# JianCao92/speaker-diarization

Hardware: AMD Instinct MI355X
Metric: diarized audio throughput (CD gw/BIC + CL hi/BIC) (higher is better)
Workload: dtype f64

## Files before the change

speaker-diarization_amd/csrc/spkd_cluster.hpp:

```cpp
#pragma once
#include "spkd_device.hpp"
#include "spkd_quad.hpp"
#include "spkd_tri.hpp"
#include "../../include/spkd.h"

namespace spkd {

constexpr double MAXINT_F = 9223372036854775808.0;
constexpr double PEN_UNIT = 39.0 + 0.5 * 39.0 * 40.0;
constexpr int AUX = 3 * DA;
constexpr int ERR_DEGENERATE_MERGE = 2;

__device__ __forceinline__ unsigned long long dkey(double v) {
    unsigned long long b = (unsigned long long)__double_as_longlong(v);
    return (b >> 63) ? ~b : (b | 0x8000000000000000ull);
}
__device__ __forceinline__ double dkey_inv(unsigned long long k) {
    unsigned long long b = (k >> 63) ? (k & 0x7fffffffffffffffull) : ~k;
    return __longlong_as_double((long long)b);
}
template <bool MAXOP>
__device__ __forceinline__ unsigned wave_red_u32(unsigned x) {
    auto op = [](unsigned a, unsigned b) { return MAXOP ? (a > b ? a : b) : (a < b ? a : b); };
    x = op(x, (unsigned)__builtin_amdgcn_update_dpp((int)x, (int)x, 0xB1, 0xf, 0xf, false));
// ... 485 lines not shown
                wmin = (wmin != wmin || d < wmin) ? d : wmin;
            }
        }
        if (variant == 1 && lane_id() == 0) {
            if (wmax == wmax) atomicMax(stat_max + p, dkey(wmax));
            if (wmin == wmin) atomicMin(stat_min + p, dkey(wmin));
        }
        return;
    }
    double* row = Dm + ra * N;
    for (int64_t base = ra + 1 + 4 * wave; base < N; base += 4 * MX_WAVES) {
        int64_t rc = base + L.m;
        const bool valid = rc < N;
        rc = valid ? rc : N - 1;
        const double det = quad_pair_det<TWO>(kind, ldsA, nA, A, ex + (off + rc) * QREC, pk + (off + rc) * REC, false, L, err);
        if (valid && L.t == 0) row[rc] = det;
    }
    __syncthreads();
    double wmax = __builtin_nan(""), wmin = __builtin_nan("");
    for (int64_t c = ra + 1 + threadIdx.x; c < N; c += MX_WAVES * WAVE) {
        const double det = row[c];
        const double nC = pk[(off + c) * REC + REC - 1];
        const double d = finish_distance(kind, lambdac, nA, ldA, nC, ld[off + c], log(det));
        row[c] = d;
        if (variant == 1) {
            Dm[c * N + ra] = d;
            if (stat_valid(d)) {
                wmax = (wmax != wmax || d > wmax) ? d : wmax;
                wmin = (wmin != wmin || d < wmin) ? d : wmin;
            }
        }
    }
    if (variant == 1) {
        const unsigned long long kmax = wave_red_u64<true>(wmax == wmax ? dkey(wmax) : 0ull);
        const unsigned long long kmin = wave_red_u64<false>(wmin == wmin ? dkey(wmin) : ~0ull);
        if (lane_id() == 0) {
            if (kmax != 0ull) atomicMax(stat_max + p, kmax);
            if (kmin != ~0ull) atomicMin(stat_min + p, kmin);
        }
    }
}

constexpr int AHC_WAVES = 8;
constexpr int AHC_TPB = AHC_WAVES * WAVE;

#ifdef SPKD_PROFILE
__device__ unsigned long long g_step_prof[8];
__device__ unsigned long long g_ahc_prof[8];
constexpr int AHC_SPAN_PROBS = 4096;
__device__ unsigned long long g_ahc_span[2 * AHC_SPAN_PROBS];
#endif
constexpr int NO_COL = 0x7fffffff;
constexpr int AHC_MAX_N = 65536;


struct RowMin { double mv; int mc, nc; };

template <class Alive>
__device__ __forceinline__ RowMin scan_row(const double* __restrict__ row, long long N, Alive alive,
                                           long long sub_col, double sub_val, int lane) {
    double mv = __builtin_huge_val();
    int mc = NO_COL, nc = NO_COL;
    for (long long c0 = 0; c0 < N; c0 += 4 * WAVE) {
        double v[4];
        int a[4];
#pragma unroll
        for (int u = 0; u < 4; ++u) {
            const long long c = c0 + u * WAVE + lane;
            const long long cc = c < N ? c : N - 1;
            a[u] = (c < N) ? (alive(cc) ? 1 : 0) : 0;
            v[u] = row[cc];
        }
#pragma unroll
        for (int u = 0; u < 4; ++u) {
            const long long cl = c0 + u * WAVE + lane;
            const int c = (int)cl;
            if (!a[u]) continue;
            const double x = (cl == sub_col) ? sub_val : v[u];
            if (x != x) { if (c < nc) nc = c; continue; }
            if (x < mv || (x == mv && c < mc)) { mv = x; mc = c; }
        }
    }
    unsigned long long okey;
    unsigned oc;
    wave_argmin_key(mc != NO_COL ? dkey(mv) : ~0ull, (unsigned)mc, okey, oc);
    RowMin r;
    r.mv = okey != ~0ull ? dkey_inv(okey) : __builtin_huge_val();
    r.mc = okey != ~0ull ? (int)oc : NO_COL;
    r.nc = __any(nc != NO_COL) ? (int)wave_red_u32<false>((unsigned)nc) : NO_COL;
    return r;
}

__device__ __forceinline__ bool row_cache_after_merge(int variant, double d, int sa, int sb,
                                                      double& rm, int& ra, int& rn) {
    if (variant != 1) return ra == sb || rn == sb;
    const bool nan_hit = rn == sa || rn == sb;
    if (ra == sa || ra == sb || nan_hit) {
        if (nan_hit || !(d < rm)) return true;
        rm = d; ra = sa;
    } else if (d != d) {
        if (sa < rn) rn = sa;
    } else if (d < rm || (d == rm && sa < ra)) {
        rm = d; ra = sa;
    }
    return false;
}
// ... 24 lines not shown
    double mx = s_tmax[0];
    if (tid == 0) {
        for (int w = 1; w < AHC_WAVES; ++w) {
            const double x = s_tmax[w];
            if (mx == mx) mx = (x != x) ? x : (x > mx ? x : mx);
        }
    }
    return mx;
}

__device__ __forceinline__ void refresh_rows(const double* __restrict__ Dm, long long N,
                                             const int32_t* __restrict__ al, int32_t* __restrict__ dirty,
                                             double* __restrict__ rmin, int32_t* __restrict__ rarg,
                                             int32_t* __restrict__ rnan, unsigned long long* masks,
                                             int tid, int wave, int lane) {
    const long long n_chunks = (N + WAVE - 1) / WAVE;
    for (long long ch = wave; ch < n_chunks; ch += AHC_WAVES) {
        const long long rl = ch * WAVE + lane;
        const long long rc = rl < N ? rl : N - 1;
        const int fa = al[rc], fd = dirty[rc];
        const unsigned long long mk = __ballot(rl < N && fa && fd);
        if (lane == 0) masks[ch] = mk;
    }
    __syncthreads();
    int ord = 0;
    for (long long ch = 0; ch < n_chunks; ++ch) {
        const long long r0 = ch * WAVE;
        unsigned long long todo = masks[ch];
        while (todo) {
            const int b = __builtin_ctzll(todo);
            todo &= todo - 1;
            if ((ord++ & (AHC_WAVES - 1)) != wave) continue;
            const long long r = r0 + b;
            const RowMin e = scan_row(Dm + r * N, N, [&](long long c) { return al[c] != 0; }, -1, 0.0, lane);
            if (lane == 0) { rmin[r] = e.mv; rarg[r] = e.mc; rnan[r] = e.nc; dirty[r] = 0; }
#ifdef SPKD_PROFILE
            if (lane == 0) atomicAdd(&g_ahc_prof[0], 1ull);
#endif
        }
    }
}

template <bool TWO>
__global__ __launch_bounds__(AHC_TPB) void k_ahc(
        double* __restrict__ ex, double* __restrict__ pk, const int64_t* __restrict__ seg_off,
        int variant, int kind, int max_spk, double lambdac, double threshold,
        double* __restrict__ ld, double* __restrict__ aux,
        double* __restrict__ mat, const int64_t* __restrict__ mat_off,
        int32_t* __restrict__ alive, double* __restrict__ tmp,
        double* __restrict__ rmin_all, int32_t* __restrict__ rcache_all,
        int32_t* __restrict__ out_n, int32_t* __restrict__ out_a, int32_t* __restrict__ out_b,
        double* __restrict__ out_d, unsigned long long* stat_max, unsigned long long* stat_min,
        double* __restrict__ final_max, double* __restrict__ final_min, int* err,
        double* pinv_ws, const int32_t* __restrict__ prob_of_block) {
    extern __shared__ int32_t ids[];
    __shared__ double ldsA[QREC];
    __shared__ unsigned long long red3[AHC_WAVES][3];
    __shared__ unsigned long long s_masks[AHC_MAX_N / WAVE];
    __shared__ int s_cnt[2];
    __shared__ int s_nids;
    __shared__ int s_next;
    __shared__ double s_tmax[AHC_WAVES];
    const int tid = threadIdx.x, lane = lane_id(), wave = tid >> 6;
    const QuadLane L = quad_lane();
    const int p = prob_of_block ? prob_of_block[blockIdx.x] : (int)blockIdx.x;
#ifdef SPKD_PROFILE
    if (tid == 0 && p < AHC_SPAN_PROBS) g_ahc_span[2 * p] = wall_clock64();
#endif
    const int64_t off = seg_off[p];
    const long long N = seg_off[p + 1] - off;
    double* Dm = mat + mat_off[p];
    int32_t* al = alive + off;
    double* ldp = ld + off;
    double* tp = tmp + off;
    double* rmin = rmin_all + off;
    int32_t* rarg = rcache_all + 3 * off;
    int32_t* rnan = rarg + N;
    int32_t* dirty = rnan + N;
    for (long long c = tid; c < N; c += AHC_TPB) { al[c] = 1; dirty[c] = 1; }
    __syncthreads();
    long long m = N;
    int n_merges = 0;
    const long long INF_IDX = 0x7fffffffffffffffLL;
    double fmin = 0.0;
#ifdef SPKD_PROFILE
    unsigned long long ahc_acc[5] = {0ull, 0ull, 0ull, 0ull, 0ull}, ahc_t = clock64();
#define AHC_TICK(i) do { const unsigned long long now_ = clock64(); ahc_acc[i] += now_ - ahc_t; ahc_t = now_; } while (0)
#else
#define AHC_TICK(i) ((void)0)
#endif
    while (true) {
        refresh_rows(Dm, N, al, dirty, rmin, rarg, rnan, s_masks, tid, wave, lane);
        __syncthreads();
        AHC_TICK(0);
        unsigned long long kb = ~0ull, ib = ~0ull, inan = ~0ull;
        for (long long r = tid; r < N; r += AHC_TPB) {
            if (!al[r]) continue;
            const double v = rmin[r];
            const int c = rarg[r], nc = rnan[r];
            if (nc != NO_COL) { const unsigned long long l = (unsigned long long)(r * N + nc); inan = l < inan ? l : inan; }
            if (c != NO_COL) {
                const unsigned long long kv = dkey(v);
                if (kv < kb) { kb = kv; ib = (unsigned long long)(r * N + c); }
            }
        }
        {
            const unsigned long long wk = wave_red_u64<false>(kb);
            const unsigned long long wi = wave_red_u64<false>(kb == wk ? ib : ~0ull);
            const unsigned long long wn = __any(inan != ~0ull) ? wave_red_u64<false>(inan) : ~0ull;
            if (lane == 0) { red3[wave][0] = wk; red3[wave][1] = wi; red3[wave][2] = wn; }
        }
        __syncthreads();
        unsigned long long bk = red3[0][0], bi = red3[0][1], bn = red3[0][2];
#pragma unroll
        for (int w = 1; w < AHC_WAVES; ++w) {
            const unsigned long long ok = red3[w][0], oi = red3[w][1], on = red3[w][2];
            const bool t = ok < bk || (ok == bk && oi < bi);
            bk = t ? ok : bk; bi = t ? oi : bi;
            bn = on < bn ? on : bn;
        }
        const bool has_nan = bn != ~0ull;
        const double mind = has_nan ? __builtin_nan("") : (bi != ~0ull ? dkey_inv(bk) : __builtin_huge_val());
        const long long index = has_nan ? (long long)bn : (bi != ~0ull ? (long long)bi : INF_IDX);
        fmin = mind;
        const bool go = (mind <= threshold) || (max_spk > 0 && m > max_spk);
        if (!go) break;
        AHC_TICK(1);
        const long long r0 = index / N, c0 = index - r0 * N;
        if (r0 == c0) {
            if (tid == 0) atomicOr(err, ERR_DEGENERATE_MERGE);
            break;
        }
        const long long sa = r0 < c0 ? r0 : c0, sb = r0 < c0 ? c0 : r0;
        if (tid < 2) s_cnt[tid] = 0;
        if (tid == 0) { s_nids = 1; s_next = 0; }
        __syncthreads();
        {
            int ca = 0, cb = 0;
            for (long long c = tid; c < sb; c += AHC_TPB) {
                if (al[c]) { cb++; if (c < sa) ca++; }
            }
            ca = __builtin_amdgcn_readlane(wave_scan_i32(ca), WAVE - 1);
            cb = __builtin_amdgcn_readlane(wave_scan_i32(cb), WAVE - 1);
            if (lane == 0 && ca) atomicAdd(&s_cnt[0], ca);
            if (lane == 0 && cb) atomicAdd(&s_cnt[1], cb);
        }
        __syncthreads();
        if (tid == 0) {
            const int64_t o = off + n_merges;
            out_a[o] = s_cnt[0]; out_b[o] = s_cnt[1]; out_d[o] = mind;
            al[sb] = 0;
            ids[0] = (int32_t)sa;
        }
        n_merges++;
        m--;
#ifdef SPKD_PROFILE
        if (tid == 0) atomicAdd(&g_ahc_prof[1], 1ull);
#endif
        double* A = ex + (off + sa) * QREC;
        const double* B = ex + (off + sb) * QREC;
        {
            double* Ap = pk + (off + sa) * REC;
            const double* Bp = pk + (off + sb) * REC;
            constexpr int NQ = (QREC + AHC_TPB - 1) / AHC_TPB, NP = (REC + AHC_TPB - 1) / AHC_TPB;
            double qa[NQ], qb[NQ], pa[NP], pb[NP];
#pragma unroll
            for (int u = 0; u < NQ; ++u) {
                const int e = tid + u * AHC_TPB;
                qa[u] = A[e < QREC ? e : 0]; qb[u] = B[e < QREC ? e : 0];
            }
#pragma unroll
            for (int u = 0; u < NP; ++u) {
                const int e = tid + u * AHC_TPB;
                pa[u] = Ap[e < REC ? e : 0]; pb[u] = Bp[e < REC ? e : 0];
            }
#pragma unroll
            for (int u = 0; u < NQ; ++u) {
                const int e = tid + u * AHC_TPB;
                const double v = qa[u] + qb[u];
                if (e < QREC) { A[e] = v; ldsA[e] = v; }
            }
#pragma unroll
            for (int u = 0; u < NP; ++u) {
                const int e = tid + u * AHC_TPB;
                if (e < REC) Ap[e] = pa[u] + pb[u];
            }
        }
        __syncthreads();
        for (long long c0 = 0; c0 < N; c0 += AHC_TPB) {
            const long long c = c0 + tid;
            const bool take = c < N && c != sa && al[c < N ? c : N - 1];
            const unsigned long long mk = __ballot(take);
            int base = 0;
            if (lane == 0 && mk) base = atomicAdd(&s_nids, __popcll(mk));
            base = __shfl(base, 0);
            if (take) ids[base + __popcll(mk & ((1ull << lane) - 1ull))] = (int32_t)c;
        }
        __syncthreads();
        AHC_TICK(2);
        const int nids = s_nids;
        const double nA = ldsA[QREC_COUNT_AT];
        if (kind == SPKD_KL2) {
            if (wave == 0) kl2_aux_from_qr(ldsA, aux + (off + sa) * AUX, pinv_ws);
        } else {
            for (;;) {
                int q4 = 0;
                if (lane == 0) q4 = atomicAdd(&s_next, 1);
                const int base = 4 * __builtin_amdgcn_readfirstlane(q4);
                if (base >= nids) break;
                int k = base + L.m;
                const bool valid = k < nids;
                k = valid ? k : nids - 1;
                const int32_t slot = ids[k];
                const double v = quad_pair_det<TWO>(kind, ldsA, nA, A, ex + (off + slot) * QREC, pk + (off + slot) * REC, k == 0, L, err);
                if (valid && L.t == 0) {
                    if (k == 0) ldp[sa] = log(v); else tp[slot] = v;
                }
            }
        }
        __syncthreads();
        AHC_TICK(3);
        double wmax = __builtin_nan(""), wmin = __builtin_nan("");
        const double ldA = ldp[sa];
        for (long long c = tid; c < N; c += AHC_TPB) {
            if (c == sa || !al[c]) continue;
            double d;
            if (kind == SPKD_KL2) {
                d = kl2_from_aux_serial(aux + (off + sa) * AUX, aux + (off + c) * AUX);
            } else {
                const double nC = qr_count(ex + (off + c) * QREC);
                d = finish_distance(kind, lambdac, nA, ldA, nC, ldp[c], log(tp[c]));
            }
            Dm[sa * N + c] = d;
            const double rm0 = rmin[c];
            const int ra0 = rarg[c], rn0 = rnan[c];
            double rm = rm0;
            int ra = ra0, rn = rn0;
            if (variant == 1) Dm[c * N + sa] = d;
            if (row_cache_after_merge(variant, d, (int)sa, (int)sb, rm, ra, rn)) dirty[c] = 1;
            else {
                if (rm != rm0 || ra != ra0) { rmin[c] = rm; rarg[c] = ra; }
                if (rn != rn0) rnan[c] = rn;
            }
            if (variant == 1 && stat_valid(d)) {
                wmax = (wmax != wmax || d > wmax) ? d : wmax;
                wmin = (wmin != wmin || d < wmin) ? d : wmin;
            }
        }
        if (tid == 0) dirty[sa] = 1;
        if (variant == 1) {
            const unsigned long long kmax = wave_red_u64<true>(wmax == wmax ? dkey(wmax) : 0ull);
            const unsigned long long kmin = wave_red_u64<false>(wmin == wmin ? dkey(wmin) : ~0ull);
            if (lane == 0) {
                if (kmax != 0ull) atomicMax(stat_max + p, kmax);
                if (kmin != ~0ull) atomicMin(stat_min + p, kmin);
            }
        }
        __syncthreads();
        AHC_TICK(4);
    }
#ifdef SPKD_PROFILE
    if (tid == 0) for (int i = 0; i < 5; ++i) atomicAdd(&g_ahc_prof[2 + i], ahc_acc[i]);
#endif
    const double mx = final_matrix_max(Dm, N, [&](long long c) { return al[c] != 0; }, s_tmax, tid);
    if (tid == 0) {
        out_n[p] = n_merges;
        final_max[p] = mx;
        final_min[p] = fmin;
#ifdef SPKD_PROFILE
        if (p < AHC_SPAN_PROBS) g_ahc_span[2 * p + 1] = wall_clock64();
#endif
    }
}

constexpr int STEP_WAVES = 4;
constexpr int STEP_WIDE_FROM = 1024;
constexpr int STEP_PARTNERS = 4 * STEP_WAVES - 1;
constexpr int ALIVE_ROUND = 0x7fffffff;
constexpr int STEP_MAX_N = 16384;
constexpr int STEP_IDX_SHIFT = 14;

struct StepState {
    int32_t done, n_merges;
    long long psa;
    double fmin;
    double diag;
};

__host__ __device__ inline unsigned long long step_slot_word(int round, int new_slot, int old_slot) {
    return ((unsigned long long)(unsigned)round << 40) | ((unsigned long long)(unsigned)new_slot << 20) |
           (unsigned long long)(unsigned)old_slot;
}
__device__ __forceinline__ int step_slot_of(unsigned long long w, int k) {
    return ((int)(w >> 40) < k) ? (int)((w >> 20) & 0xfffffull) : (int)(w & 0xfffffull);
}

struct StepSel {
    double rmin, newrow;
    int32_t rarg, rnan, death, pad;
};

struct StepArrays {
    double* ex;
    double* pk;
    double* exm;
    double* pkm;
    int32_t* death;
    StepSel* sel2;
    unsigned long long* sw;
    double* cnt;
    StepState* state2;
// ... 574 lines not shown
```

speaker-diarization_amd/csrc/spkd_hip.hip:

```cpp
#include <hip/hip_runtime.h>

#include <algorithm>
#include <cmath>
#include <cstddef>
#include <cstdio>
#include <cstdlib>
#include <cstring>
#include <functional>
#include <string>
#include <atomic>
#include <thread>
#include <vector>

#include "../../include/spkd.h"
#include "spkd_cd.hpp"
#include "spkd_cluster.hpp"
#include "spkd_device.hpp"
#include "spkd_handoff.hpp"
#include "spkd_merge.hpp"
#include "spkd_stats.hpp"
#include "spkd_post_stats.hpp"
#include "spkd_mfcc.hpp"
#include "spkd_mfcc_batch.hpp"
#include "spkd_resample.hpp"
#include "spkd_vad.hpp"
#include "spkd_vad_batch.hpp"
#include "spkd_mindur.hpp"
#include "spkd_fb.hpp"
#include "spkd_gauss.hpp"
#include "spkd_gmm_train.hpp"
#include "spkd_ubm_stats.hpp"
#include "spkd_clr.hpp"
#include "spkd_ident.hpp"

using namespace spkd;

namespace {
constexpr int N_SLOTS = 72;
enum { PIN_GW_TURNS = 0, PIN_GW_LINES, PIN_AHC_OUT, PIN_VAD_FILES, PIN_VAD_TOKENS, PIN_SUM_IDX, PIN_GAUSS_IDX,
       PIN_GT_TAB, PIN_GT_OUT, PIN_GT_IDX, PIN_UBM_TAB, PIN_UBM_OUT, PIN_CLR_IN, PIN_CLR_OUT, PIN_MD_SEQS, PIN_MD_TOKENS,
       PIN_FB_TAB, PIN_ID_IN, PIN_ID_OUT, PIN_ACC_TAB, PIN_POST_TAB, N_PIN };
}

struct spkd_ctx {
    int device = 0;
    hipStream_t stream = nullptr;
    bool own_stream = false;
    bool gw_lds_ok = false;
    int rs_lds_cap = 0;
    int gw_waves = 0;
    unsigned long long init_keys[2] = {0ull, ~0ull};
    int step_waves = 0;
    int step_partners = 0;
    int64_t last_gw_items = 0;
    int ahc_head = -1;
    int64_t last_ahc_head = 0;
    hipStream_t side = nullptr;
    hipEvent_t ev_fork = nullptr, ev_join = nullptr;
    std::string err;
    int* d_err = nullptr;
    unsigned long long* d_counter = nullptr;
    hipEvent_t ev0 = nullptr, ev1 = nullptr;
    float last_ms = 0.f;
    hipEvent_t ka[SPKD_N_TIMERS] = {}, kb[SPKD_N_TIMERS] = {};
    bool kused[SPKD_N_TIMERS] = {};
    float kms[SPKD_N_TIMERS] = {};
    void* slot[N_SLOTS] = {};
    size_t slot_bytes[N_SLOTS] = {};
    void* pinv_ws = nullptr;
    double* pinv_cur = nullptr;
    void* pin[N_PIN] = {};
    size_t pin_bytes[N_PIN] = {};
    std::vector<int64_t> redo_line, redo_begin, redo_end;
    std::vector<Chunk> redo_chunks;
    std::vector<int64_t> redo_setoff;
    std::vector<int32_t> redo_sets;
};

namespace {

spkd_status fail(spkd_ctx* c, spkd_status s, const std::string& msg) {
    if (c) c->err = msg;
    return s;
}

#define HIPCHK(c, call)                                                              \
    do {                                                                             \
        hipError_t e_ = (call);                                                      \
        if (e_ != hipSuccess)                                                        \
            return fail((c), SPKD_EHIP, std::string(#call) + ": " + hipGetErrorString(e_)); \
    } while (0)

#define TRY(expr) do { const spkd_status s_ = (expr); if (s_ != SPKD_OK) return s_; } while (0)

spkd_status scratch(spkd_ctx* c, int slot, size_t bytes, void** out) {
    if (bytes == 0) bytes = 16;
    if (c->slot_bytes[slot] < bytes) {
        if (c->slot[slot]) HIPCHK(c, hipFree(c->slot[slot]));
        c->slot[slot] = nullptr;
        c->slot_bytes[slot] = 0;
        size_t want = bytes + bytes / 4;
        hipError_t e = hipMalloc(&c->slot[slot], want);
        if (e != hipSuccess) {
            want = bytes;
            e = hipMalloc(&c->slot[slot], want);
        }
        if (e != hipSuccess) return fail(c, SPKD_ENOMEM, "scratch allocation failed");
        c->slot_bytes[slot] = want;
    }
// ... 194 lines not shown
    S_MD_TAB, S_MD_BACK, S_MD_G, S_MD_B, S_MD_SEQS, S_MD_TOKENS, S_FB_TAB, S_FB_FWD, S_FB_OUT,
    S_ID_WORK, S_ID_MAT, S_ACC_TAB, S_POST_TAB, S_POST_PARTIAL, S_RS_TAB, S_COUNT
};
static_assert(S_COUNT <= N_SLOTS, "scratch slot table too small");

}

extern "C" {

int spkd_abi_version(void) { return SPKD_ABI_VERSION; }

static spkd_status create_ctx(int device, void* stream, bool borrow, spkd_ctx** out) {
    if (!out) return SPKD_EINVAL;
    *out = nullptr;
    int count = 0;
    if (hipGetDeviceCount(&count) != hipSuccess || device < 0 || device >= count) return SPKD_EHIP;
    spkd_ctx* c = new spkd_ctx();
    c->device = device;
    if (hipSetDevice(device) != hipSuccess) { delete c; return SPKD_EHIP; }
    if (borrow) {
        c->stream = (hipStream_t)stream;
    } else {
        if (hipStreamCreateWithFlags(&c->stream, hipStreamDefault) != hipSuccess) { delete c; return SPKD_EHIP; }
        c->own_stream = true;
    }
    if (hipMalloc(&c->d_err, sizeof(int)) != hipSuccess ||
        hipMalloc(&c->d_counter, 2 * sizeof(unsigned long long)) != hipSuccess ||
        hipEventCreate(&c->ev0) != hipSuccess || hipEventCreate(&c->ev1) != hipSuccess) {
        spkd_destroy(c);
        return SPKD_EHIP;
    }
    for (int i = 0; i < SPKD_N_TIMERS; ++i)
        if (hipEventCreate(&c->ka[i]) != hipSuccess || hipEventCreate(&c->kb[i]) != hipSuccess) {
            spkd_destroy(c);
            return SPKD_EHIP;
        }
    int lds_max = 0;
    c->gw_lds_ok = hipDeviceGetAttribute(&lds_max, hipDeviceAttributeMaxSharedMemoryPerBlock, device) == hipSuccess &&
                   Gw<4>::LDS_BYTES <= lds_max &&
                   hipFuncSetAttribute((const void*)k_gw<8>, hipFuncAttributeMaxDynamicSharedMemorySize, Gw<8>::LDS_BYTES) == hipSuccess &&
                   hipFuncSetAttribute((const void*)k_gw<4>, hipFuncAttributeMaxDynamicSharedMemorySize, Gw<4>::LDS_BYTES) == hipSuccess &&
                   hipFuncSetAttribute((const void*)k_gw<2>, hipFuncAttributeMaxDynamicSharedMemorySize, Gw<2>::LDS_BYTES) == hipSuccess &&
                   hipFuncSetAttribute((const void*)k_gw<1>, hipFuncAttributeMaxDynamicSharedMemorySize, Gw<1>::LDS_BYTES) == hipSuccess;
    c->rs_lds_cap = 64 * 1024;
    if (lds_max > c->rs_lds_cap) {
        const int want = lds_max < RS_LDS_MAX ? lds_max : RS_LDS_MAX;
        if (hipFuncSetAttribute((const void*)k_resample, hipFuncAttributeMaxDynamicSharedMemorySize, want) == hipSuccess)
            c->rs_lds_cap = want;
    }
    if (const char* e = getenv("SPKD_GW_WAVES")) c->gw_waves = atoi(e);
    if (const char* e = getenv("SPKD_STEP_WAVES")) { const int v = atoi(e); c->step_waves = (v == 4 || v == 8) ? v : 0; }
    if (const char* e = getenv("SPKD_STEP_PARTNERS")) { const int v = atoi(e); c->step_partners = (v == 3 || v == 7 || v == 15) ? v : 0; }
    if (const char* e = getenv("SPKD_AHC_HEAD")) { const int v = atoi(e); c->ahc_head = v >= 0 ? v : -1; }
    *out = c;
    return SPKD_OK;
}

spkd_status spkd_create(int device, void* stream, spkd_ctx** out) {
    return create_ctx(device, stream, stream != nullptr, out);
}

spkd_status spkd_create_on_stream(int device, void* stream, spkd_ctx** out) {
    return create_ctx(device, stream, true, out);
}

void spkd_destroy(spkd_ctx* c) {
    if (!c) return;
    (void)hipSetDevice(c->device);
    if (c->stream) (void)hipStreamSynchronize(c->stream);
    if (c->side) {
        (void)hipStreamSynchronize(c->side);
        (void)hipStreamDestroy(c->side);
    }
    if (c->ev_fork) (void)hipEventDestroy(c->ev_fork);
    if (c->ev_join) (void)hipEventDestroy(c->ev_join);
    for (int i = 0; i < N_SLOTS; ++i)
        if (c->slot[i]) (void)hipFree(c->slot[i]);
    if (c->d_err) (void)hipFree(c->d_err);
    if (c->pinv_ws) (void)hipFree(c->pinv_ws);
    for (int i = 0; i < N_PIN; ++i)
        if (c->pin[i]) (void)hipHostFree(c->pin[i]);
    if (c->d_counter) (void)hipFree(c->d_counter);
    if (c->ev0) (void)hipEventDestroy(c->ev0);
    if (c->ev1) (void)hipEventDestroy(c->ev1);
    for (int i = 0; i < SPKD_N_TIMERS; ++i) {
        if (c->ka[i]) (void)hipEventDestroy(c->ka[i]);
        if (c->kb[i]) (void)hipEventDestroy(c->kb[i]);
    }
    if (c->own_stream && c->stream) (void)hipStreamDestroy(c->stream);
    delete c;
}

const char* spkd_last_error(const spkd_ctx* c) { return c ? c->err.c_str() : "null context"; }

spkd_status spkd_sync(spkd_ctx* c) {
    if (!c) return SPKD_EINVAL;
    HIPCHK(c, hipStreamSynchronize(c->stream));
    return SPKD_OK;
}

spkd_status spkd_malloc(spkd_ctx* c, size_t bytes, void** d_ptr) {
    if (!c || !d_ptr) return SPKD_EINVAL;
    HIPCHK(c, hipSetDevice(c->device));
    hipError_t e = hipMalloc(d_ptr, bytes ? bytes : 16);
    if (e != hipSuccess) return fail(c, SPKD_ENOMEM, hipGetErrorString(e));
    return SPKD_OK;
// ... 172 lines not shown
    }
    size_t longest = 0;
    for (auto& l : lists) longest = std::max(longest, l.size());
    sched.assign(longest * X, -1);
    for (int x = 0; x < X; ++x)
        for (size_t i = 0; i < lists[x].size(); ++i) sched[i * X + x] = lists[x][i];
    if (by_xcd) {
        by_xcd->clear();
        for (size_t i = 0; by_xcd->size() < order.size(); ++i)
            for (int x = 0; x < X; ++x) if (i < probs[x].size()) by_xcd->push_back(probs[x][i]);
    }
}

unsigned long long host_dkey(double v) {
    unsigned long long b;
    std::memcpy(&b, &v, sizeof b);
    return (b >> 63) ? ~b : (b | 0x8000000000000000ull);
}

struct MatrixPlan {
    const double* d_init = nullptr;
    double init_max = NAN, init_min = NAN;
    int64_t row_begin = -1, row_end = -1;
    int64_t* d_map = nullptr;
    int64_t n_src = 0;
    const float* d_frames = nullptr;
    int64_t n_frames = 0;
    const int64_t *redo_line = nullptr, *redo_begin = nullptr, *redo_end = nullptr;
    int64_t n_redo = 0;
};

void to_quadrec(spkd_ctx* c, const double* d_stats, int64_t n, double* ex) {
    hipLaunchKernelGGL(k_to_quadrec, dim3((unsigned)n), dim3(256), 0, c->stream, d_stats, n, ex);
}

void cluster_prep(spkd_ctx* c, const double* ex, int64_t n, int kind, double* ld, double* aux) {
    const int64_t per_block = kind == SPKD_KL2 ? PT_WAVES : 4 * PT_WAVES;
    const unsigned blocks = (unsigned)((n + per_block - 1) / per_block);
    hipLaunchKernelGGL(k_cluster_prep, dim3(blocks), dim3(PT_WAVES * WAVE), 0, c->stream, ex, n, kind, ld, aux, c->d_err,
                       c->pinv_cur);
}

void matrix_launch(spkd_ctx* c, const AhcPrep& B, const int32_t* d_sched, int64_t grid) {
    if (grid <= 0) return;
    auto kmat = B.kind == SPKD_GLR ? k_matrix<true> : k_matrix<false>;
    hipLaunchKernelGGL(kmat, dim3((unsigned)grid), dim3(MX_WAVES * WAVE), 0, c->stream,
                       (const double*)B.ex, (const double*)B.pk, (const int64_t*)B.seg_off, (const int32_t*)B.d_prob,
                       d_sched, B.variant, B.kind, B.lambdac,
                       (const double*)B.ld, (const double*)B.aux, B.mat, (const int64_t*)B.mat_off,
                       B.smax, B.smin, c->d_err);
}

constexpr int AHC_HEAD_ROUND = 32;
constexpr double AHC_MS_PER_N2 = 2.122e-4;
constexpr double MATRIX_MS_PER_N2 = 5.58e-7;
constexpr int AHC_HEAD_MAX = 32;
constexpr int AHC_RULE_CUS = 256;
int64_t ahc_head_rule(const std::vector<int64_t>& n, int cus) {
    const int64_t n_prob = (int64_t)n.size();
    if (n_prob < 16) return 0;
    auto t = [](int64_t N) { return AHC_MS_PER_N2 * (double)N * (double)N; };
    double sum_all = 0.0;
    for (int64_t N : n) sum_all += (double)N * (double)N;
    const double stage0 = MATRIX_MS_PER_N2 * sum_all + t(n[0]);
    double best = stage0, sum_head = 0.0;
    int64_t best_k = 0;
    for (int64_t k = 1; k <= std::min<int64_t>(AHC_HEAD_MAX, n_prob) && k < cus; ++k) {
        sum_head += (double)n[(size_t)k - 1] * (double)n[(size_t)k - 1];
        const double m_head = MATRIX_MS_PER_N2 * sum_head, m_rest = MATRIX_MS_PER_N2 * (sum_all - sum_head);
        const double rest = k < n_prob ? m_rest * cus / (double)(cus - k) + t(n[(size_t)k]) : 0.0;
        const double stage = m_head + std::max(t(n[0]), rest);
        if (k % AHC_HEAD_ROUND == 0 && stage < best) { best = stage; best_k = k; }
    }
    return stage0 - best < 0.01 * stage0 ? 0 : best_k;
}

spkd_status ahc_prepare(spkd_ctx* c, const double* d_stats, const int64_t* h_seg_off, int64_t n_prob,
                        int variant, int kind, double lambdac, AhcPrep& B, const MatrixPlan& plan = MatrixPlan()) {
    const int64_t n_total = B.n_total = h_seg_off[n_prob];
    const size_t np = (size_t)n_prob;
    std::vector<int64_t> mat_off(np + 1);
    int64_t cells = 0;
    for (int64_t p = 0; p < n_prob; ++p) {
        const int64_t n = h_seg_off[p + 1] - h_seg_off[p];
        if (n < 0) return fail(c, SPKD_EINVAL, "seg_off must be non-decreasing");
        mat_off[(size_t)p] = cells;
        cells += n * n;
    }
    mat_off[np] = cells;
    std::vector<int32_t> prob((size_t)n_total, 0);
    for (int64_t p = 0; p < n_prob; ++p)
        for (int64_t r = h_seg_off[p]; r < h_seg_off[p + 1]; ++r) prob[(size_t)r] = (int32_t)p;
    {
        std::vector<int32_t> sched, sched_head, block_head, block_rest;
        if (plan.row_begin >= 0) {
            const int64_t rows = plan.row_end - plan.row_begin;
            sched.assign((size_t)((rows + N_XCD - 1) / N_XCD * N_XCD), -1);
            for (int64_t i = 0; i < rows; ++i) sched[(size_t)i] = (int32_t)(plan.row_begin + i);
        } else {
            std::vector<int64_t> order((size_t)n_prob);
            for (int64_t p = 0; p < n_prob; ++p) order[(size_t)p] = p;
            std::stable_sort(order.begin(), order.end(), [&](int64_t a, int64_t b) {
                return h_seg_off[a + 1] - h_seg_off[a] > h_seg_off[b + 1] - h_seg_off[b];
            });
            const std::vector<int64_t> head(order.begin(), order.begin() + B.head_k), rest(order.begin() + B.head_k, order.end());
            deal_to_xcds(h_seg_off, rest, sched);
            if (B.head_k > 0) {
                deal_to_xcds(h_seg_off, head, sched_head, &block_head);
// ... 231 lines not shown
        h_n_clusters[p] = done2[2 * p + 1];
    }
    return st;
}

spkd_status spkd_distance_rows(spkd_ctx* c, int variant, int kind, double lambdac, const double* d_stats,
                               int64_t n, int64_t row_begin, int64_t row_end, double* d_rows,
                               double* h_stat_max, double* h_stat_min) {
    if (!c || n < 0 || bad_kind(kind) || (variant != 1 && variant != 2)) return SPKD_EINVAL;
    if (row_begin < 0 || row_end < row_begin || row_end > n) return fail(c, SPKD_EINVAL, "distance_rows: bad row block");
    if (h_stat_max) *h_stat_max = std::nan("");
    if (h_stat_min) *h_stat_min = std::nan("");
    if (n == 0 || row_end == row_begin) return SPKD_OK;
    if (!d_stats || !d_rows) return fail(c, SPKD_EINVAL, "null argument");
    const int64_t seg_off[2] = {0, n};
    AhcPrep B;
    MatrixPlan plan;
    plan.row_begin = row_begin;
    plan.row_end = row_end;
    unsigned long long keys[2] = {0ull, ~0ull};
    Call call(c);
    TRY(call.opened);
    TRY(use_kind(c, kind, &kind));
    TRY(ahc_prepare(c, d_stats, seg_off, 1, variant, kind, lambdac, B, plan));
    HIPCHK(c, hipMemcpyAsync(d_rows, B.mat + row_begin * n, (size_t)(row_end - row_begin) * n * sizeof(double),
                             hipMemcpyDeviceToDevice, c->stream));
    HIPCHK(c, hipMemcpyAsync(&keys[0], B.smax, sizeof(unsigned long long), hipMemcpyDeviceToHost, c->stream));
    HIPCHK(c, hipMemcpyAsync(&keys[1], B.smin, sizeof(unsigned long long), hipMemcpyDeviceToHost, c->stream));
    const spkd_status st = call.finish();
    if (h_stat_max) *h_stat_max = key_to_double(keys[0], true);
    if (h_stat_min) *h_stat_min = key_to_double(keys[1], false);
    return st;
}

namespace {
spkd_status ahc_impl(spkd_ctx* c, const double* d_stats, const int64_t* h_seg_off, int64_t n_prob,
                     const spkd_ahc_params* P, const MatrixPlan& plan, int32_t* h_n_merges, int32_t* h_merge_a,
                     int32_t* h_merge_b, double* h_merge_d, double* h_stat_max, double* h_stat_min) {
    if (!c || !P || n_prob < 0) return SPKD_EINVAL;
    if (n_prob == 0) return SPKD_OK;
    if (!d_stats || !h_seg_off || !h_n_merges || !h_merge_a || !h_merge_b || !h_merge_d ||
        !h_stat_max || !h_stat_min)
        return fail(c, SPKD_EINVAL, "null argument");
    if ((P->variant != 1 && P->variant != 2) || bad_kind(P->kind))
        return fail(c, SPKD_EINVAL, "bad variant / kind");
    for (int64_t p = 0; p < n_prob; ++p)
        if (h_seg_off[p + 1] - h_seg_off[p] < 1) return fail(c, SPKD_EINVAL, "empty clustering problem");
    int64_t n_max = 0;
    for (int64_t p = 0; p < n_prob; ++p) n_max = std::max<int64_t>(n_max, h_seg_off[p + 1] - h_seg_off[p]);
    if (n_max > AHC_MAX_N) return fail(c, SPKD_EINVAL, "clustering problem larger than 65536 records");
    int path = P->path;
    if (path != SPKD_AHC_MONO && path != SPKD_AHC_WIDE) path = n_prob <= 64 ? SPKD_AHC_WIDE : SPKD_AHC_MONO;
    const size_t lds = (size_t)(n_max + 4) * sizeof(int32_t);
    if (path == SPKD_AHC_MONO && lds > 150 * 1024) path = SPKD_AHC_WIDE;
    if (path == SPKD_AHC_WIDE && n_max > STEP_MAX_N)
        return fail(c, SPKD_EINVAL, "clustering problem larger than 16384 records (wide merge loop)");
    AhcPrep B;
    c->last_ahc_head = 0;
    if (path == SPKD_AHC_MONO && !plan.d_init && plan.row_begin < 0 && P->kind != SPKD_KL2_PINV) {
        B.head_k = c->ahc_head >= 0 ? std::min<int64_t>(c->ahc_head, n_prob) : spkd_ahc_head_rule(h_seg_off, n_prob);
        c->last_ahc_head = B.head_k;
    }
    std::vector<unsigned long long> kmax((size_t)n_prob), kmin((size_t)n_prob);
    std::vector<double> fmax((size_t)n_prob), fmin((size_t)n_prob);
    Call call(c);
    TRY(call.opened);
    spkd_ahc_params Pk;
    TRY(kernel_params(c, P, Pk));
    TRY(ahc_prepare(c, d_stats, h_seg_off, n_prob, P->variant, P->kind, P->lambdac, B, plan));
    const int64_t n_total = B.n_total;
    const size_t nt = (size_t)n_total, np = (size_t)n_prob;
    double *d_merge_d, *d_tmp, *d_rmin, *d_fmax, *d_fmin;
    int32_t *d_a, *d_b, *d_alive, *d_rcache, *d_n;
    TRY(carve(c, scratch, S_AHC_OUT, [&](Layout L) {
        return L.part(d_merge_d, nt).part(d_tmp, nt).part(d_rmin, nt).part(d_fmax, np).part(d_fmin, np)
            .part(d_a, nt).part(d_b, nt).part(d_alive, nt).part(d_rcache, 3 * nt).part(d_n, np).bytes();
    }));
    if (path == SPKD_AHC_MONO) {
        auto kahc = P->kind == SPKD_GLR ? k_ahc<true> : k_ahc<false>;
        if (lds > 48 * 1024)
            (void)hipFuncSetAttribute((const void*)kahc, hipFuncAttributeMaxDynamicSharedMemorySize, (int)lds);
        auto merge_loops = [&](hipStream_t on, int64_t grid, const int32_t* blocks, int64_t largest) {
            hipLaunchKernelGGL(kahc, dim3((unsigned)grid), dim3(AHC_TPB), (size_t)(largest + 4) * sizeof(int32_t), on,
                               B.ex, B.pk, (const int64_t*)B.seg_off, P->variant, P->kind, P->max_spk, P->lambdac,
                               P->threshold, B.ld, B.aux, B.mat, (const int64_t*)B.mat_off, d_alive, d_tmp,
                               d_rmin, d_rcache, d_n, d_a, d_b, d_merge_d, B.smax, B.smin, d_fmax, d_fmin, c->d_err,
                               c->pinv_cur, blocks);
        };
        if (B.head_k > 0) {
            TRY(call.fork());
            (void)hipEventRecord(c->ka[SPKD_T_AHC], c->side);
            merge_loops(c->side, B.head_k, B.d_block_head, B.n_max_head);
            matrix_launch(c, B, B.d_sched, B.grid_rows);
            (void)hipEventRecord(c->kb[SPKD_T_MATRIX], c->stream);
            c->kused[SPKD_T_MATRIX] = true;
            if (n_prob > B.head_k) merge_loops(c->stream, n_prob - B.head_k, B.d_block_rest, B.n_max_rest);
            HIPCHK(c, hipGetLastError());
            TRY(call.join());
            (void)hipEventRecord(c->kb[SPKD_T_AHC], c->stream);
            c->kused[SPKD_T_AHC] = true;
        } else {
            Timer t(c, SPKD_T_AHC);
            merge_loops(c->stream, n_prob, nullptr, n_max);
        }
    } else {
        StepArrays Q;
        void *pe = nullptr, *pp = nullptr;
        TRY(carve(c, scratch, S_STEP_MISC, [&](Layout L) {
            return L.part(Q.sel2, 2 * nt).part(Q.cnt, nt).part(Q.sw, nt).part(Q.state2, 2 * np).part(Q.death, nt).bytes();
        }));
        TRY(scratch(c, S_STEP_EXM, nt * QREC * sizeof(double), &pe));
        TRY(scratch(c, S_STEP_PKM, nt * REC * sizeof(double), &pp));
        Q.ex = B.ex; Q.pk = B.pk; Q.exm = (double*)pe; Q.pkm = (double*)pp;
        Q.n_total = n_total;
        Q.n_prob = (int32_t)n_prob;
        const int step_waves = c->step_waves ? c->step_waves : (n_max > STEP_WIDE_FROM ? 8 : 4);
        const bool glr_k = P->kind == SPKD_GLR;
        using StepKernel = decltype(&k_ahc_step<false, 4, 3>);
        StepKernel kvar[3];
        if (step_waves == 8) {
            kvar[0] = glr_k ? k_ahc_step<true, 8, 3> : k_ahc_step<false, 8, 3>;
            kvar[1] = glr_k ? k_ahc_step<true, 8, 7> : k_ahc_step<false, 8, 7>;
            kvar[2] = glr_k ? k_ahc_step<true, 8, STEP_PARTNERS> : k_ahc_step<false, 8, STEP_PARTNERS>;
        } else {
            kvar[0] = glr_k ? k_ahc_step<true, 4, 3> : k_ahc_step<false, 4, 3>;
            kvar[1] = glr_k ? k_ahc_step<true, 4, 7> : k_ahc_step<false, 4, 7>;
            kvar[2] = glr_k ? k_ahc_step<true, 4, STEP_PARTNERS> : k_ahc_step<false, 4, STEP_PARTNERS>;
        }
        auto sp_of_round = [&](int64_t partners) -> int {
            if (c->step_partners) return c->step_partners;
            const int64_t free_cus = 255;
            if (partners * n_prob <= 3 * free_cus) return 3;
            if (partners * n_prob <= 7 * free_cus) return 7;
            return STEP_PARTNERS;
        };
        const size_t nch_max = (size_t)((n_max + WAVE - 1) / WAVE);
        const size_t step_lds = ((size_t)2 * n_max + nch_max + 2) * sizeof(int32_t) + nch_max * sizeof(unsigned long long);
        if (step_lds + 20 * 1024 > 48 * 1024)
            for (int v = 0; v < 3; ++v)
                (void)hipFuncSetAttribute((const void*)kvar[v], hipFuncAttributeMaxDynamicSharedMemorySize, (int)step_lds);
// ... 2293 lines not shown
```

Before: 1610.

## Carry AHC row minima across merges to skip refresh and global argmin scan

In the monolithic AHC merge loop, the merged row's minimum is now built from per-thread partial minima during the distance update, and the global argmin is updated in the same pass. When no other row's cached minimum is invalidated, the next iteration skips refresh_rows and the full rmin scan and reuses the carried candidate. The merged row's cache entry is written later, overlapped with the next merge's record loads. This adds LDS for per-thread partials, recomputes the LDS budget used for path selection, and retunes the head-split cost constants.

New measurement: 1624, median of 6. About the same (+0.9%).

```diff
diff --git a/speaker-diarization_amd/csrc/spkd_cluster.hpp b/speaker-diarization_amd/csrc/spkd_cluster.hpp
--- a/speaker-diarization_amd/csrc/spkd_cluster.hpp
+++ b/speaker-diarization_amd/csrc/spkd_cluster.hpp
@@ -561,6 +561,9 @@
 #endif
 constexpr int NO_COL = 0x7fffffff;
 constexpr int AHC_MAX_N = 65536;
+constexpr int AHC_STATIC_LDS = QREC * 8 + AHC_WAVES * 3 * 8 + (AHC_MAX_N / WAVE) * 8 + AHC_WAVES * WAVE * 16 +
+                               AHC_WAVES * 12 + 16 + 256;
+constexpr int AHC_IDS_LDS_MAX = 160 * 1024 - AHC_STATIC_LDS;
 
 
 struct RowMin { double mv; int mc, nc; };
@@ -691,7 +694,7 @@
         int32_t* __restrict__ out_n, int32_t* __restrict__ out_a, int32_t* __restrict__ out_b,
         double* __restrict__ out_d, unsigned long long* stat_max, unsigned long long* stat_min,
         double* __restrict__ final_max, double* __restrict__ final_min, int* err,
-        double* pinv_ws, const int32_t* __restrict__ prob_of_block) {
+        double* pinv_ws, const int32_t* __restrict__ prob_of_block, int carry) {
     extern __shared__ int32_t ids[];
     __shared__ double ldsA[QREC];
     __shared__ unsigned long long red3[AHC_WAVES][3];
@@ -700,6 +703,8 @@
     __shared__ int s_nids;
     __shared__ int s_next;
     __shared__ double s_tmax[AHC_WAVES];
+    __shared__ alignas(16) RowMin s_part[AHC_TPB];
+    __shared__ int s_went[AHC_WAVES];
     const int tid = threadIdx.x, lane = lane_id(), wave = tid >> 6;
     const QuadLane L = quad_lane();
     const int p = prob_of_block ? prob_of_block[blockIdx.x] : (int)blockIdx.x;
@@ -728,19 +733,50 @@
 #else
 #define AHC_TICK(i) ((void)0)
 #endif
+    bool carried = false;
+    unsigned long long ckb = ~0ull, cib = ~0ull, cnan = ~0ull;
+    long long pend_sa = -1;
+    auto row_sa_lane = [&]() {
+        RowMin r = s_part[lane];
+#pragma unroll
+        for (int w = 1; w < AHC_WAVES; ++w) {
+            const RowMin x = s_part[w * WAVE + lane];
+            const bool take = x.mv < r.mv || (x.mv == r.mv && x.mc < r.mc);
+            r.mv = take ? x.mv : r.mv;
+            r.mc = take ? x.mc : r.mc;
+            r.nc = x.nc < r.nc ? x.nc : r.nc;
+        }
+        return r;
+    };
+    auto row_sa_entry = [&]() {
+        const RowMin x = row_sa_lane();
+        unsigned long long okey;
+        unsigned oc;
+        wave_argmin_key(x.mc != NO_COL ? dkey(x.mv) : ~0ull, (unsigned)x.mc, okey, oc);
+        RowMin e;
+        e.mv = okey != ~0ull ? dkey_inv(okey) : __builtin_huge_val();
+        e.mc = okey != ~0ull ? (int)oc : NO_COL;
+        e.nc = __any(x.nc != NO_COL) ? (int)wave_red_u32<false>((unsigned)x.nc) : NO_COL;
+        return e;
+    };
     while (true) {
-        refresh_rows(Dm, N, al, dirty, rmin, rarg, rnan, s_masks, tid, wave, lane);
-        __syncthreads();
+        if (!carried) {
+            refresh_rows(Dm, N, al, dirty, rmin, rarg, rnan, s_masks, tid, wave, lane);
+            __syncthreads();
+        }
         AHC_TICK(0);
-        unsigned long long kb = ~0ull, ib = ~0ull, inan = ~0ull;
-        for (long long r = tid; r < N; r += AHC_TPB) {
-            if (!al[r]) continue;
-            const double v = rmin[r];
-            const int c = rarg[r], nc = rnan[r];
-            if (nc != NO_COL) { const unsigned long long l = (unsigned long long)(r * N + nc); inan = l < inan ? l : inan; }
-            if (c != NO_COL) {
-                const unsigned long long kv = dkey(v);
-                if (kv < kb) { kb = kv; ib = (unsigned long long)(r * N + c); }
+        unsigned long long kb = ckb, ib = cib, inan = cnan;
+        if (!carried) {
+            kb = ib = inan = ~0ull;
+            for (long long r = tid; r < N; r += AHC_TPB) {
+                if (!al[r]) continue;
+                const double v = rmin[r];
+                const int c = rarg[r], nc = rnan[r];
+                if (nc != NO_COL) { const unsigned long long l = (unsigned long long)(r * N + nc); inan = l < inan ? l : inan; }
+                if (c != NO_COL) {
+                    const unsigned long long kv = dkey(v);
+                    if (kv < kb) { kb = kv; ib = (unsigned long long)(r * N + c); }
+                }
             }
         }
         {
@@ -812,6 +848,10 @@
             for (int u = 0; u < NP; ++u) {
                 const int e = tid + u * AHC_TPB;
                 pa[u] = Ap[e < REC ? e : 0]; pb[u] = Bp[e < REC ? e : 0];
+            }
+            if (pend_sa >= 0 && wave == AHC_WAVES - 1) {
+                const RowMin e = row_sa_entry();
+                if (lane == 0) { rmin[pend_sa] = e.mv; rarg[pend_sa] = e.mc; rnan[pend_sa] = e.nc; }
             }
 #pragma unroll
             for (int u = 0; u < NQ; ++u) {
@@ -861,8 +901,21 @@
         AHC_TICK(3);
         double wmax = __builtin_nan(""), wmin = __builtin_nan("");
         const double ldA = ldp[sa];
+        const double diag = carry ? Dm[sa * N + sa] : 0.0;
+        double pmv = __builtin_huge_val();
+        int pmc = NO_COL, pnc = NO_COL;
+        auto to_row_sa = [&pmv, &pmc, &pnc](double x, int c) {
+            const bool isnan = x != x;
+            const bool take = x < pmv || (x == pmv && c < pmc);
+            pnc = isnan && c < pnc ? c : pnc;
+            pmv = take ? x : pmv;
+            pmc = take ? c : pmc;
+        };
+        bool went = false;
+        ckb = cib = cnan = ~0ull;
         for (long long c = tid; c < N; c += AHC_TPB) {
-            if (c == sa || !al[c]) continue;
+            if (c == sa) { if (carry) to_row_sa(diag, (int)c); continue; }
+            if (!al[c]) continue;
             double d;
             if (kind == SPKD_KL2) {
                 d = kl2_from_aux_serial(aux + (off + sa) * AUX, aux + (off + c) * AUX);
@@ -876,17 +929,31 @@
             double rm = rm0;
             int ra = ra0, rn = rn0;
             if (variant == 1) Dm[c * N + sa] = d;
-            if (row_cache_after_merge(variant, d, (int)sa, (int)sb, rm, ra, rn)) dirty[c] = 1;
+            if (row_cache_after_merge(variant, d, (int)sa, (int)sb, rm, ra, rn)) { dirty[c] = 1; went = true; }
             else {
                 if (rm != rm0 || ra != ra0) { rmin[c] = rm; rarg[c] = ra; }
                 if (rn != rn0) rnan[c] = rn;
-            }
+                if (rn != NO_COL) { const unsigned long long l = (unsigned long long)(c * N + rn); cnan = l < cnan ? l : cnan; }
+                if (ra != NO_COL) {
+                    const unsigned long long kv = dkey(rm);
+                    if (kv < ckb) { ckb = kv; cib = (unsigned long long)(c * N + ra); }
+                }
+            }
+            if (carry) to_row_sa(d, (int)c);
             if (variant == 1 && stat_valid(d)) {
                 wmax = (wmax != wmax || d > wmax) ? d : wmax;
                 wmin = (wmin != wmin || d < wmin) ? d : wmin;
             }
         }
-        if (tid == 0) dirty[sa] = 1;
+        if (carry) {
+            RowMin part;
+            part.mv = pmv; part.mc = pmc; part.nc = pnc;
+            int t = tid;
+            asm volatile("" : "+v"(t));
+            s_part[t] = part;
+            const bool w = __any(went);
+            if ((t & (WAVE - 1)) == 0) s_went[t >> 6] = w ? 1 : 0;
+        } else if (tid == 0) dirty[sa] = 1;
         if (variant == 1) {
             const unsigned long long kmax = wave_red_u64<true>(wmax == wmax ? dkey(wmax) : 0ull);
             const unsigned long long kmin = wave_red_u64<false>(wmin == wmin ? dkey(wmin) : ~0ull);
@@ -896,6 +963,32 @@
             }
         }
         __syncthreads();
+        if (carry) {
+            int any = 0;
+#pragma unroll
+            for (int w = 0; w < AHC_WAVES; ++w) any |= s_went[w];
+            carried = !any;
+            if (!carried) {
+                if (wave == 0) {
+                    const RowMin e = row_sa_entry();
+                    if (lane == 0) { rmin[sa] = e.mv; rarg[sa] = e.mc; rnan[sa] = e.nc; }
+                }
+                pend_sa = -1;
+            } else {
+                if (wave == 0) {
+                    const RowMin x = row_sa_lane();
+                    if (x.nc != NO_COL) { const unsigned long long l = (unsigned long long)(sa * N + x.nc); cnan = l < cnan ? l : cnan; }
+                    const unsigned long long kv = x.mc != NO_COL ? dkey(x.mv) : ~0ull, l = (unsigned long long)(sa * N + x.mc);
+                    const bool take = x.mc != NO_COL && (kv < ckb || (kv == ckb && l < cib));
+                    ckb = take ? kv : ckb;
+                    cib = take ? l : cib;
+                }
+                pend_sa = sa;
+#ifdef SPKD_PROFILE
+                if (tid == 0) atomicAdd(&g_ahc_prof[7], 1ull);
+#endif
+            }
+        }
         AHC_TICK(4);
     }
 #ifdef SPKD_PROFILE
diff --git a/speaker-diarization_amd/csrc/spkd_hip.hip b/speaker-diarization_amd/csrc/spkd_hip.hip
--- a/speaker-diarization_amd/csrc/spkd_hip.hip
+++ b/speaker-diarization_amd/csrc/spkd_hip.hip
@@ -55,6 +55,7 @@
     int64_t last_gw_items = 0;
     int ahc_head = -1;
     int64_t last_ahc_head = 0;
+    int ahc_carry = 1;
     hipStream_t side = nullptr;
     hipEvent_t ev_fork = nullptr, ev_join = nullptr;
     std::string err;
@@ -355,6 +356,7 @@
     if (const char* e = getenv("SPKD_STEP_WAVES")) { const int v = atoi(e); c->step_waves = (v == 4 || v == 8) ? v : 0; }
     if (const char* e = getenv("SPKD_STEP_PARTNERS")) { const int v = atoi(e); c->step_partners = (v == 3 || v == 7 || v == 15) ? v : 0; }
     if (const char* e = getenv("SPKD_AHC_HEAD")) { const int v = atoi(e); c->ahc_head = v >= 0 ? v : -1; }
+    if (const char* e = getenv("SPKD_AHC_CARRY")) c->ahc_carry = atoi(e) != 0 ? 1 : 0;
     *out = c;
     return SPKD_OK;
 }
@@ -633,8 +635,8 @@
 }
 
 constexpr int AHC_HEAD_ROUND = 32;
-constexpr double AHC_MS_PER_N2 = 2.122e-4;
-constexpr double MATRIX_MS_PER_N2 = 5.58e-7;
+constexpr double AHC_MS_PER_N2 = 2.052e-4;
+constexpr double MATRIX_MS_PER_N2 = 5.45e-7;
 constexpr int AHC_HEAD_MAX = 32;
 constexpr int AHC_RULE_CUS = 256;
 int64_t ahc_head_rule(const std::vector<int64_t>& n, int cus) {
@@ -972,7 +974,7 @@
     int path = P->path;
     if (path != SPKD_AHC_MONO && path != SPKD_AHC_WIDE) path = n_prob <= 64 ? SPKD_AHC_WIDE : SPKD_AHC_MONO;
     const size_t lds = (size_t)(n_max + 4) * sizeof(int32_t);
-    if (path == SPKD_AHC_MONO && lds > 150 * 1024) path = SPKD_AHC_WIDE;
+    if (path == SPKD_AHC_MONO && lds > (size_t)AHC_IDS_LDS_MAX) path = SPKD_AHC_WIDE;
     if (path == SPKD_AHC_WIDE && n_max > STEP_MAX_N)
         return fail(c, SPKD_EINVAL, "clustering problem larger than 16384 records (wide merge loop)");
     AhcPrep B;
@@ -1005,7 +1007,7 @@
                                B.ex, B.pk, (const int64_t*)B.seg_off, P->variant, P->kind, P->max_spk, P->lambdac,
                                P->threshold, B.ld, B.aux, B.mat, (const int64_t*)B.mat_off, d_alive, d_tmp,
                                d_rmin, d_rcache, d_n, d_a, d_b, d_merge_d, B.smax, B.smin, d_fmax, d_fmin, c->d_err,
-                               c->pinv_cur, blocks);
+                               c->pinv_cur, blocks, c->ahc_carry);
         };
         if (B.head_k > 0) {
             TRY(call.fork());
```
